# finegrain-ai/refiners

Hardware: NVIDIA B200
Metric: SDXL 1024^2 bf16 denoising steps/s (latent batch 8, CFG, Euler) (higher is better)
Workload: dtype bf16

## Files before the change

### refiners_b200/csrc/tc_attention2.cu

```cuda
#include <cuda.h>

#include <cstdlib>

#include "common.cuh"
#include "tc_ptx.cuh"

namespace rb200 {
namespace {

using namespace ptx;

constexpr int QT = 128;
constexpr int KT = 128;
constexpr int HD = 64;
constexpr int STAGES = 2;
constexpr int NUM_THREADS = 640;
constexpr int Q_TILE_BYTES = QT * HD * 2;
constexpr int Q_BYTES = 2 * Q_TILE_BYTES;
constexpr int K_BYTES = KT * HD * 2, V_BYTES = KT * HD * 2;
constexpr int P_SLAB = QT * 64 * 2;
constexpr int P_BYTES = 2 * P_SLAB;
constexpr int TMEM_COLS = 512;
constexpr int XCHG_BYTES = 2  * 2  * 2  * QT * 4;
constexpr size_t SMEM_BYTES = 2 * Q_BYTES + STAGES * (K_BYTES + V_BYTES) + 2 * P_BYTES + 1024  + 256  + XCHG_BYTES;
static_assert(SMEM_BYTES <= 227 * 1024, "exceeds the 227 KB of shared memory a CTA can opt in to");
constexpr float RESCALE_LOG2 = 8.0f;

struct Attn2Params {
  void* o;
  int64_t o_sb, o_ss;
  int H;
  int64_t Sq, Sk;
  int n_pairs;
  int64_t total_work;
  int ntiles;
  float scale_log2e;
  uint32_t idesc_qk, idesc_pv;
  int d_out;
  int stagger;
};

template <typename T> __device__ __forceinline__ uint32_t pack2(float a, float b);
template <> __device__ __forceinline__ uint32_t pack2<__nv_bfloat16>(float a, float b) {
  __nv_bfloat162 v = __floats2bfloat162_rn(a, b);
  return *reinterpret_cast<uint32_t*>(&v);
}
template <> __device__ __forceinline__ uint32_t pack2<__half>(float a, float b) {
  __half2 v = __floats2half2_rn(a, b);
  return *reinterpret_cast<uint32_t*>(&v);
}

template <typename T, int POLY>
__global__ void __launch_bounds__(NUM_THREADS, 1)
tc_sdpa2_kernel(const __grid_constant__ CUtensorMap map_q, const __grid_constant__ CUtensorMap map_k,
                const __grid_constant__ CUtensorMap map_v, const Attn2Params p) {
  extern __shared__ uint8_t smem_raw[];
  uint8_t* smem = reinterpret_cast<uint8_t*>((reinterpret_cast<uintptr_t>(smem_raw) + 1023) & ~uintptr_t(1023));
  uint8_t* sQ = smem;
  uint8_t* sK = sQ + 2 * Q_BYTES;
  uint8_t* sV = sK + STAGES * K_BYTES;
  uint8_t* sP = sV + STAGES * V_BYTES;
  uint64_t* bars = reinterpret_cast<uint64_t*>(sP + 2 * P_BYTES);
  uint64_t* kv_full = bars;
  uint64_t* kv_empty = bars + STAGES;
  uint64_t* q_full = bars + 2 * STAGES;
  uint64_t* q_empty = q_full + 2;
  uint64_t* bar_s = q_full + 4;
  uint64_t* bar_sfree = q_full + 6;
  uint64_t* bar_p = q_full + 8;
  uint64_t* bar_o = q_full + 10;
  uint64_t* bar_ofree = q_full + 12;
  uint32_t* tmem_slot = reinterpret_cast<uint32_t*>(q_full + 14);
  float* xchg = reinterpret_cast<float*>(reinterpret_cast<uint8_t*>(bars) + 256);

  const int warp = threadIdx.x >> 5, lane = threadIdx.x & 31;
  const int wg = warp >> 2;

  if (warp == 0 && lane == 0) {
    prefetch_tmap(&map_q);
    prefetch_tmap(&map_k);
    prefetch_tmap(&map_v);
    for (int s = 0; s < STAGES; ++s) {
      mbar_init(&kv_full[s], 1);
      mbar_init(&kv_empty[s], 2);
    }
    for (int b = 0; b < 2; ++b) {
      mbar_init(&q_full[b], 1);
      mbar_init(&q_empty[b], 2);
      mbar_init(&bar_s[b], 1);
      mbar_init(&bar_sfree[b], 8);
      mbar_init(&bar_p[b], 8);
      mbar_init(&bar_o[b], 1);
      mbar_init(&bar_ofree[b], 8);
    }
    fence_barrier_init();
  }
  if (warp == 1) tmem_alloc<TMEM_COLS>(tmem_slot);
  tcgen05_fence_before();
  __syncthreads();
  tcgen05_fence_after();
  const uint32_t tmem_base = *tmem_slot;

  if (wg == 0) {
    setmaxnreg_dec<56>();
    if (warp == 0) {
      if (lane == 0) {
        int stage = 0;
        uint32_t phase = 0;
        uint32_t n = 0;
        for (int64_t w = blockIdx.x; w < p.total_work; w += gridDim.x, ++n) {
          const int pair = int(w % p.n_pairs);
          const int h = int((w / p.n_pairs) % p.H);
          const int b = int(w / (int64_t(p.n_pairs) * p.H));
          const uint32_t qb = n & 1, qph = (n >> 1) & 1;
          mbar_wait(&q_empty[qb], qph ^ 1, 1);
          mbar_arrive_expect_tx(&q_full[qb], Q_BYTES);
          tma_load_4d(sQ + qb * Q_BYTES, &map_q, &q_full[qb], 0, h, pair * 2 * QT, b);
          tma_load_4d(sQ + qb * Q_BYTES + Q_TILE_BYTES, &map_q, &q_full[qb], 0, h, pair * 2 * QT + QT, b);
          for (int j = 0; j < p.ntiles; ++j) {
            mbar_wait(&kv_empty[stage], phase ^ 1, 2);
            mbar_arrive_expect_tx(&kv_full[stage], K_BYTES + V_BYTES);
            tma_load_4d(sK + stage * K_BYTES, &map_k, &kv_full[stage], 0, h, j * KT, b);
            tma_load_4d(sV + stage * V_BYTES, &map_v, &kv_full[stage], 0, h, j * KT, b);
            if (++stage == STAGES) {
              stage = 0;
              phase ^= 1;
            }
          }
        }
      }
    } else if (warp == 1 || warp == 2) {
      if (lane == 0) {
        const int g = warp - 1;
        int st_k = 0, st_v = 0;
        uint32_t ph_k = 0;
        uint32_t t = 0;
        uint32_t s_issued = 0;
        uint32_t n = 0;
        const uint32_t tmem_s = tmem_base + g * 128, tmem_o = tmem_base + 256 + g * 64;
        const uint32_t pbase = smem_u32(sP + g * P_BYTES);
        auto issue_s = [&](uint32_t qb, int stage_k) {
          if (s_issued > 0) mbar_wait(&bar_sfree[g], (s_issued - 1) & 1, 4);
          ++s_issued;
          tcgen05_fence_after();
          const uint64_t dq = desc_kmajor(smem_u32(sQ + qb * Q_BYTES + g * Q_TILE_BYTES));
          const uint64_t dk = desc_kmajor(smem_u32(sK + stage_k * K_BYTES));
#pragma unroll
          for (int k = 0; k < HD / 16; ++k) umma_f16(tmem_s, dq + uint64_t(k * 2), dk + uint64_t(k * 2), p.idesc_qk, k > 0);
          umma_commit(&bar_s[g]);
        };
        auto next_k = [&]() {
          if (++st_k == STAGES) {
            st_k = 0;
            ph_k ^= 1;
          }
        };
        for (int64_t w = blockIdx.x; w < p.total_work; w += gridDim.x, ++n) {
          const uint32_t qb = n & 1, qph = (n >> 1) & 1;
          mbar_wait(&q_full[qb], qph, 5);
          mbar_wait(&kv_full[st_k], ph_k, 3);
          issue_s(qb, st_k);
          next_k();
          for (int j = 0; j < p.ntiles; ++j) {
            if (j + 1 < p.ntiles) {
              mbar_wait(&kv_full[st_k], ph_k, 6);
              issue_s(qb, st_k);
              next_k();
            }
            mbar_wait(&bar_p[g], t & 1, 7);
            if (j == 0 && n > 0) mbar_wait(&bar_ofree[g], (n - 1) & 1, 8);
            tcgen05_fence_after();
            const uint32_t vbase = smem_u32(sV + st_v * V_BYTES);
#pragma unroll
            for (int k = 0; k < KT / 16; ++k) {
              const uint64_t dp = desc_kmajor(pbase + (k >> 2) * P_SLAB) + uint64_t((k & 3) * 2);
              const uint64_t dv = desc_mnmajor(vbase, V_BYTES) + uint64_t(k * 128);
              umma_f16(tmem_o, dp, dv, p.idesc_pv, (j > 0 || k > 0) ? 1u : 0u);
            }
            umma_commit(&kv_empty[st_v]);
            umma_commit(&bar_o[g]);
            ++t;
            if (++st_v == STAGES) st_v = 0;
          }
          umma_commit(&q_empty[qb]);
        }
      }
    }
  } else {
    setmaxnreg_inc<104>();
    const int g = (wg - 1) >> 1;
    const int hf = (wg - 1) & 1;
    const int lg = warp & 3;
    const int row = lg * 32 + lane;
    const uint32_t lane_off = uint32_t(lg * 32) << 16;
    const uint32_t tmem_s = tmem_base + g * 128 + hf * 64 + lane_off;
    const uint32_t tmem_o = tmem_base + 256 + g * 64 + hf * 32 + lane_off;
    const uint32_t prow = smem_u32(sP + g * P_BYTES + hf * P_SLAB + row * 128);
    const int sw = row & 7;
    const uint32_t xg = smem_u32(xchg + g * (2 * 2 * QT));
    const uint32_t x_mine = xg + uint32_t(hf * QT + row) * 4, x_other = xg + uint32_t((hf ^ 1) * QT + row) * 4;
    const uint32_t a_s = smem_u32(&bar_s[g]), a_sfree = smem_u32(&bar_sfree[g]), a_p = smem_u32(&bar_p[g]);
    const uint32_t a_o = smem_u32(&bar_o[g]), a_ofree = smem_u32(&bar_ofree[g]);
    const uint32_t swz = uint32_t(sw) << 4;
    const uint32_t xbar = 1 + g;
    T* obase = static_cast<T*>(p.o);
    uint32_t t = 0;
    uint32_t n = 0;
    for (int64_t w = blockIdx.x; w < p.total_work; w += gridDim.x, ++n) {
      const int pair = int(w % p.n_pairs);
      const int h = int((w / p.n_pairs) % p.H);
      const int64_t b = w / (int64_t(p.n_pairs) * p.H);
      float m_run = -INFINITY, l_run = 0.f;
      for (int j = 0; j < p.ntiles; ++j, ++t) {
        mbar_wait_a(a_s, t & 1);
        tcgen05_fence_after();
        float s[KT / 2];
        {
          uint32_t r0[32], r1[32];
          tmem_ld_32x32(tmem_s, r0);
          tmem_ld_32x32(tmem_s + 32, r1);
          tmem_ld_wait();
#pragma unroll
          for (int i = 0; i < 32; ++i) {
            s[i] = __uint_as_float(r0[i]);
            s[32 + i] = __uint_as_float(r1[i]);
          }
        }
        tcgen05_fence_before();
        __syncwarp();
        if (lane == 0) mbar_arrive_relaxed_a(a_sfree);
        const int64_t left = p.Sk - int64_t(j) * KT - hf * 64;
        if (left < 64) {
          const int valid = left > 0 ? int(left) : 0;
#pragma unroll
          for (int i = 0; i < 64; ++i)
            if (i >= valid) s[i] = -INFINITY;
        }
        float tm0 = fmaxf(s[0], s[1]), tm1 = fmaxf(s[2], s[3]), tm2 = fmaxf(s[4], s[5]), tm3 = fmaxf(s[6], s[7]);
#pragma unroll
        for (int i = 8; i < 64; i += 8) {
          tm0 = fmaxf(tm0, fmaxf(s[i], s[i + 1]));
          tm1 = fmaxf(tm1, fmaxf(s[i + 2], s[i + 3]));
          tm2 = fmaxf(tm2, fmaxf(s[i + 4], s[i + 5]));
          tm3 = fmaxf(tm3, fmaxf(s[i + 6], s[i + 7]));
        }
        const uint32_t slot = (t & 1) * (2 * QT * 4);
        const float mine = fmaxf(fmaxf(tm0, tm1), fmaxf(tm2, tm3));
        st_shared_f32(x_mine + slot, mine);
        named_bar_sync(xbar, 256);
        const float tmax = fmaxf(mine, ld_shared_f32(x_other + slot));
        bool waited_o = false;
        if (j == 0) {
          m_run = tmax;
        } else {
          const float m_new = fmaxf(m_run, tmax);
          const bool grew = (m_new - m_run) * p.scale_log2e > RESCALE_LOG2;
          if (__any_sync(0xffffffffu, grew)) {
            mbar_wait_a(a_o, (t - 1) & 1);
            waited_o = true;
            tcgen05_fence_after();
            const float alpha = ex2_approx((m_run - m_new) * p.scale_log2e);
            uint32_t raw[32];
            tmem_ld_32x32(tmem_o, raw);
            tmem_ld_wait();
#pragma unroll
            for (int i = 0; i < 32; ++i) raw[i] = __float_as_uint(__uint_as_float(raw[i]) * alpha);
            tmem_st_32x32(tmem_o, raw);
            tmem_st_wait();
            l_run *= alpha;
            m_run = m_new;
          }
        }
        const float mb = m_run * p.scale_log2e;
        if ((j > 0 && !waited_o) || (j == 0 && t > 0)) mbar_wait_a(a_o, (t - 1) & 1);
        if (p.stagger == 1) {
          if (g == 1 && j == 0) named_bar_sync(3, 512);
        } else if (p.stagger == 2) {
          if (g == 1) named_bar_sync(3, 512);
          else if (t > 0) named_bar_sync(4, 512);
        }
        const uint64_t sc2 = f32x2(p.scale_log2e, p.scale_log2e), nmb2 = f32x2(-mb, -mb);
        uint64_t sum_a = f32x2(0.f, 0.f), sum_b = sum_a;
#pragma unroll
        for (int c = 0; c < 8; ++c) {
          uint32_t pk[4];
#pragma unroll
          for (int q = 0; q < 2; ++q) {
            const int i = c * 8 + q * 4;
            float x0, x1, x2, x3;
            f32x2_split(fma_f32x2(f32x2(s[i], s[i + 1]), sc2, nmb2), x0, x1);
            f32x2_split(fma_f32x2(f32x2(s[i + 2], s[i + 3]), sc2, nmb2), x2, x3);
            const float p0 = ex2_approx(x0), p2 = ex2_approx(x2);
            const float p1 = POLY >= 2 ? ex2_poly(x1) : ex2_approx(x1);
            const float p3 = POLY >= 1 ? ex2_poly(x3) : ex2_approx(x3);
            sum_a = add_f32x2(sum_a, f32x2(p0, p1));
            sum_b = add_f32x2(sum_b, f32x2(p2, p3));
            pk[q * 2] = pack2<T>(p0, p1);
            pk[q * 2 + 1] = pack2<T>(p2, p3);
          }
          st_shared_v4(prow + ((uint32_t(c) << 4) ^ swz), pk[0], pk[1], pk[2], pk[3]);
        }
        {
          float a0, a1;
          f32x2_split(add_f32x2(sum_a, sum_b), a0, a1);
          l_run += a0 + a1;
        }
        if (p.stagger == 1) {
          if (g == 0 && j == 0) named_bar_arrive(3, 512);
        } else if (p.stagger == 2) {
          named_bar_arrive(g == 0 ? 3 : 4, 512);
        }
        fence_proxy_async();
        tcgen05_fence_before();
        __syncwarp();
        if (lane == 0) mbar_arrive_a(a_p);
      }
      const uint32_t slot = (t & 1) * (2 * QT * 4);
      st_shared_f32(x_mine + slot, l_run);
      named_bar_sync(xbar, 256);
      const float l_row = l_run + ld_shared_f32(x_other + slot);
      named_bar_sync(xbar, 256);
      mbar_wait_a(a_o, (t - 1) & 1);
      tcgen05_fence_after();
      const float inv = l_row > 0.f ? 1.f / l_row : 0.f;
      float acc[32];
      {
        uint32_t raw[32];
        tmem_ld_32x32(tmem_o, raw);
        tmem_ld_wait();
#pragma unroll
        for (int i = 0; i < 32; ++i) acc[i] = inv * __uint_as_float(raw[i]);
      }
      tcgen05_fence_before();
      __syncwarp();
      if (lane == 0) mbar_arrive_relaxed_a(a_ofree);
      const int64_t qi = (int64_t(pair) * 2 + g) * QT + row;
      if (qi < p.Sq) {
        T* dst = obase + b * p.o_sb + qi * p.o_ss + int64_t(h) * p.d_out + hf * 32;
        if ((reinterpret_cast<uintptr_t>(dst) & 15) == 0 && (p.d_out & 7) == 0) {
#pragma unroll
          for (int c = 0; c < 4; ++c) {
            if (hf * 32 + c * 8 >= p.d_out) break;
            uint4 v;
            v.x = pack2<T>(acc[c * 8], acc[c * 8 + 1]);
            v.y = pack2<T>(acc[c * 8 + 2], acc[c * 8 + 3]);
            v.z = pack2<T>(acc[c * 8 + 4], acc[c * 8 + 5]);
            v.w = pack2<T>(acc[c * 8 + 6], acc[c * 8 + 7]);
            reinterpret_cast<uint4*>(dst)[c] = v;
          }
        } else {
#pragma unroll
          for (int i = 0; i < 32; ++i)
            if (hf * 32 + i < p.d_out) dst[i] = from_f<T>(acc[i]);
        }
      }
    }
  }

  tcgen05_fence_before();
  __syncthreads();
  if (warp == 1) {
    tcgen05_fence_after();
    tmem_dealloc<TMEM_COLS>(tmem_base);
  }
}

typedef CUresult (*EncodeTiledFn)(CUtensorMap*, CUtensorMapDataType, cuuint32_t, void*, const cuuint64_t*, const cuuint64_t*,
                                  const cuuint32_t*, const cuuint32_t*, CUtensorMapInterleave, CUtensorMapSwizzle,
                                  CUtensorMapL2promotion, CUtensorMapFloatOOBfill);
EncodeTiledFn encode_fn() {
  static EncodeTiledFn fn = [] {
    void* sym = nullptr;
    cudaDriverEntryPointQueryResult q;
    if (cudaGetDriverEntryPoint("cuTensorMapEncodeTiled", &sym, cudaEnableDefault, &q) != cudaSuccess || q != cudaDriverEntryPointSuccess)
      return EncodeTiledFn(nullptr);
    return reinterpret_cast<EncodeTiledFn>(sym);
  }();
  return fn;
}

int make_map(CUtensorMap* map, int dtype, const void* base, int64_t B, int64_t S, int H, int64_t sb, int64_t ss, int D) {
  EncodeTiledFn fn = encode_fn();
  if (!fn) RB200_FAIL(-4, "cuTensorMapEncodeTiled unavailable");
  const cuuint64_t dims[4] = {cuuint64_t(D), cuuint64_t(H), cuuint64_t(S), cuuint64_t(B)};
  const cuuint64_t strides[3] = {cuuint64_t(D) * 2, cuuint64_t(ss) * 2, cuuint64_t(sb) * 2};
  const cuuint32_t box[4] = {64, 1, 128, 1};
  const cuuint32_t es[4] = {1, 1, 1, 1};
  const CUtensorMapDataType dt = dtype == RB200_BF16 ? CU_TENSOR_MAP_DATA_TYPE_BFLOAT16 : CU_TENSOR_MAP_DATA_TYPE_FLOAT16;
  CUresult rc = fn(map, dt, 4, const_cast<void*>(base), dims, strides, box, es, CU_TENSOR_MAP_INTERLEAVE_NONE,
                   CU_TENSOR_MAP_SWIZZLE_128B, CU_TENSOR_MAP_L2_PROMOTION_L2_256B, CU_TENSOR_MAP_FLOAT_OOB_FILL_NONE);
  if (rc != CUDA_SUCCESS) RB200_FAIL(-4, "sdpa2 tensor map encode failed (%d): S=%lld H=%d ss=%lld sb=%lld", int(rc), (long long)S, H, (long long)ss, (long long)sb);
  return 0;
}

bool ok_operand(const void* ptr, int64_t sb, int64_t ss) {
  return (reinterpret_cast<uintptr_t>(ptr) & 15) == 0 && ss % 8 == 0 && sb % 8 == 0;
}

template <typename T, int POLY>
int launch(cudaStream_t st, const CUtensorMap& mq, const CUtensorMap& mk, const CUtensorMap& mv, const Attn2Params& prm) {
  static PerDeviceOnce configured;
  if (configured.needed()) {
    if (cudaFuncSetAttribute(tc_sdpa2_kernel<T, POLY>, cudaFuncAttributeMaxDynamicSharedMemorySize, int(SMEM_BYTES)) != cudaSuccess)
      RB200_FAIL(-2, "tc_sdpa2: cannot reserve %zu bytes of shared memory", SMEM_BYTES);
    configured.done();
  }
  const int64_t cap = sm_count();
  const int grid = int(prm.total_work < cap ? prm.total_work : cap);
  tc_sdpa2_kernel<T, POLY><<<grid, NUM_THREADS, SMEM_BYTES, st>>>(mq, mk, mv, prm);
  RB200_CHECK_LAUNCH("tc_sdpa2");
  return 0;
}

int env_int(const char* name, int fallback) {
  const char* e = getenv(name);
  return e ? atoi(e) : fallback;
}

}

bool tc_sdpa2_supported(const SdpaProblem& p) {
  static const int enabled = env_int("RB200_ATTN_V2", 1);
  if (!enabled) return false;
  if (p.dtype != RB200_BF16 && p.dtype != RB200_FP16) return false;
  if (p.D < 8 || p.D > 64 || (p.D & 7) != 0 || p.causal) return false;
  if (p.bias_h != nullptr || (p.k2 != nullptr && p.Sk2 > 0)) return false;
  if (p.Sq <= QT || p.Sk <= KT || p.B < 1) return false;
  return ok_operand(p.q, p.q_sb, p.q_ss) && ok_operand(p.k, p.k_sb, p.k_ss) && ok_operand(p.v, p.v_sb, p.v_ss);
}

int tc_sdpa2(cudaStream_t st, const SdpaProblem& p) {
  CUtensorMap mq, mk, mv;
  if (int rc = make_map(&mq, p.dtype, p.q, p.B, p.Sq, p.H, p.q_sb, p.q_ss, p.D)) return rc;
  if (int rc = make_map(&mk, p.dtype, p.k, p.B, p.Sk, p.H, p.k_sb, p.k_ss, p.D)) return rc;
  if (int rc = make_map(&mv, p.dtype, p.v, p.B, p.Sk, p.H, p.v_sb, p.v_ss, p.D)) return rc;
  Attn2Params prm{};
  prm.o = p.o;
  prm.o_sb = p.o_sb;
  prm.o_ss = p.o_ss;
  prm.H = p.H;
  prm.Sq = p.Sq;
  prm.Sk = p.Sk;
  prm.n_pairs = int(ceil_div(p.Sq, 2 * QT));
  prm.total_work = int64_t(prm.n_pairs) * p.H * p.B;
  prm.ntiles = int(ceil_div(p.Sk, KT));
  prm.scale_log2e = p.scale * 1.4426950408889634f;
  const uint32_t fmt = p.dtype == RB200_BF16 ? 1u : 0u;
  const uint32_t common = (1u << 4) | (fmt << 7) | (fmt << 10) | (uint32_t(QT >> 4) << 24);
  prm.idesc_qk = common | (uint32_t(KT >> 3) << 17);
  prm.idesc_pv = common | (uint32_t(HD >> 3) << 17) | (1u << 16);
  prm.d_out = p.D;
  static const int stagger = env_int("RB200_ATTN_STAGGER", 2);
  prm.stagger = stagger;
  static const int poly = env_int("RB200_ATTN_POLY", 0);
  const bool bf = p.dtype == RB200_BF16;
  if (poly >= 2) return bf ? launch<__nv_bfloat16, 2>(st, mq, mk, mv, prm) : launch<__half, 2>(st, mq, mk, mv, prm);
  if (poly == 1) return bf ? launch<__nv_bfloat16, 1>(st, mq, mk, mv, prm) : launch<__half, 1>(st, mq, mk, mv, prm);
  return bf ? launch<__nv_bfloat16, 0>(st, mq, mk, mv, prm) : launch<__half, 0>(st, mq, mk, mv, prm);
}

}
```

### refiners_b200/csrc/tc_ptx.cuh

```cuda
#pragma once

#include <cuda.h>
#include <stdint.h>


namespace rb200 {
namespace ptx {

static __device__ __forceinline__ uint32_t smem_u32(const void* p) { return static_cast<uint32_t>(__cvta_generic_to_shared(p)); }

static __device__ __forceinline__ void mbar_init(uint64_t* bar, uint32_t count) {
  asm volatile("mbarrier.init.shared::cta.b64 [%0], %1;" ::"r"(smem_u32(bar)), "r"(count));
}
static __device__ __forceinline__ void fence_barrier_init() { asm volatile("fence.mbarrier_init.release.cluster;" ::: "memory"); }
static __device__ __forceinline__ void mbar_arrive_expect_tx(uint64_t* bar, uint32_t bytes) {
  asm volatile("mbarrier.arrive.expect_tx.shared::cta.b64 _, [%0], %1;" ::"r"(smem_u32(bar)), "r"(bytes) : "memory");
}
static __device__ __forceinline__ void mbar_arrive(uint64_t* bar) {
  asm volatile("mbarrier.arrive.shared::cta.b64 _, [%0];" ::"r"(smem_u32(bar)) : "memory");
}
static __device__ __forceinline__ void mbar_arrive_relaxed(uint64_t* bar) {
  asm volatile("mbarrier.arrive.relaxed.cta.shared::cta.b64 _, [%0];" ::"r"(smem_u32(bar)) : "memory");
}
static __device__ __forceinline__ bool mbar_try_wait(uint64_t* bar, uint32_t parity) {
  uint32_t ok;
  asm volatile(
      "{\n\t.reg .pred p;\n\t"
      "mbarrier.try_wait.parity.shared::cta.b64 p, [%1], %2;\n\t"
      "selp.u32 %0, 1, 0, p;\n\t}"
      : "=r"(ok)
      : "r"(smem_u32(bar)), "r"(parity)
      : "memory");
  return ok != 0;
}
static __device__ __forceinline__ void mbar_wait(uint64_t* bar, uint32_t parity, int tag = 0) {
  (void)tag;
  for (uint32_t spin = 0; !mbar_try_wait(bar, parity); ++spin) {
    if (spin > (1u << 26)) __trap();
  }
}

static __device__ __forceinline__ void mbar_arrive_a(uint32_t bar) {
  asm volatile("mbarrier.arrive.shared::cta.b64 _, [%0];" ::"r"(bar) : "memory");
}
static __device__ __forceinline__ void mbar_arrive_relaxed_a(uint32_t bar) {
  asm volatile("mbarrier.arrive.relaxed.cta.shared::cta.b64 _, [%0];" ::"r"(bar) : "memory");
}
static __device__ __forceinline__ bool mbar_try_wait_a(uint32_t bar, uint32_t parity) {
  uint32_t ok;
  asm volatile(
      "{\n\t.reg .pred p;\n\t"
      "mbarrier.try_wait.parity.shared::cta.b64 p, [%1], %2;\n\t"
      "selp.u32 %0, 1, 0, p;\n\t}"
      : "=r"(ok)
      : "r"(bar), "r"(parity)
      : "memory");
  return ok != 0;
}
static __device__ __forceinline__ void mbar_wait_a(uint32_t bar, uint32_t parity) {
  for (uint32_t spin = 0; !mbar_try_wait_a(bar, parity); ++spin) {
    if (spin > (1u << 26)) __trap();
  }
}
static __device__ __forceinline__ float ld_shared_f32(uint32_t addr) {
  float v;
  asm volatile("ld.shared.f32 %0, [%1];" : "=f"(v) : "r"(addr) : "memory");
  return v;
}
static __device__ __forceinline__ void st_shared_f32(uint32_t addr, float v) {
  asm volatile("st.shared.f32 [%0], %1;" ::"r"(addr), "f"(v) : "memory");
}

static __device__ __forceinline__ uint64_t f32x2(float lo, float hi) {
  uint64_t r;
  asm("mov.b64 %0, {%1, %2};" : "=l"(r) : "f"(lo), "f"(hi));
  return r;
}
static __device__ __forceinline__ void f32x2_split(uint64_t v, float& lo, float& hi) {
  asm("mov.b64 {%0, %1}, %2;" : "=f"(lo), "=f"(hi) : "l"(v));
}
static __device__ __forceinline__ uint64_t fma_f32x2(uint64_t a, uint64_t b, uint64_t c) {
  uint64_t d;
  asm("fma.rn.f32x2 %0, %1, %2, %3;" : "=l"(d) : "l"(a), "l"(b), "l"(c));
  return d;
}
static __device__ __forceinline__ uint64_t add_f32x2(uint64_t a, uint64_t b) {
  uint64_t d;
  asm("add.rn.f32x2 %0, %1, %2;" : "=l"(d) : "l"(a), "l"(b));
  return d;
}

static __device__ __forceinline__ void prefetch_tmap(const CUtensorMap* map) {
  asm volatile("prefetch.tensormap [%0];" ::"l"(reinterpret_cast<uint64_t>(map)) : "memory");
}
static __device__ __forceinline__ void tma_load_4d(void* dst, const CUtensorMap* map, uint64_t* bar, int c0, int c1, int c2, int c3) {
  asm volatile(
      "cp.async.bulk.tensor.4d.shared::cluster.global.mbarrier::complete_tx::bytes [%0], [%1, {%3, %4, %5, %6}], [%2];"
      ::"r"(smem_u32(dst)), "l"(reinterpret_cast<uint64_t>(map)), "r"(smem_u32(bar)), "r"(c0), "r"(c1), "r"(c2), "r"(c3)
      : "memory");
}
static __device__ __forceinline__ void fence_proxy_async() { asm volatile("fence.proxy.async.shared::cta;" ::: "memory"); }

static __device__ __forceinline__ void tcgen05_fence_before() { asm volatile("tcgen05.fence::before_thread_sync;" ::: "memory"); }
static __device__ __forceinline__ void tcgen05_fence_after() { asm volatile("tcgen05.fence::after_thread_sync;" ::: "memory"); }

template <int COLS>
static __device__ __forceinline__ void tmem_alloc(uint32_t* dst_smem) {
  asm volatile("tcgen05.alloc.cta_group::1.sync.aligned.shared::cta.b32 [%0], %1;" ::"r"(smem_u32(dst_smem)), "n"(COLS) : "memory");
  asm volatile("tcgen05.relinquish_alloc_permit.cta_group::1.sync.aligned;" ::: "memory");
}
template <int COLS>
static __device__ __forceinline__ void tmem_dealloc(uint32_t addr) {
  asm volatile("tcgen05.dealloc.cta_group::1.sync.aligned.b32 %0, %1;" ::"r"(addr), "n"(COLS) : "memory");
}

static __device__ __forceinline__ void umma_f16(uint32_t tmem_d, uint64_t desc_a, uint64_t desc_b, uint32_t idesc, uint32_t accumulate) {
  asm volatile(
      "{\n\t.reg .pred p;\n\t"
      "setp.ne.b32 p, %4, 0;\n\t"
      "tcgen05.mma.cta_group::1.kind::f16 [%0], %1, %2, %3, p;\n\t}"
      ::"r"(tmem_d), "l"(desc_a), "l"(desc_b), "r"(idesc), "r"(accumulate)
      : "memory");
}
static __device__ __forceinline__ void umma_commit(uint64_t* bar) {
  asm volatile("tcgen05.commit.cta_group::1.mbarrier::arrive::one.shared::cluster.b64 [%0];" ::"r"(smem_u32(bar)) : "memory");
}

static __device__ __forceinline__ void tmem_ld_32x32(uint32_t taddr, uint32_t (&r)[32]) {
  asm volatile(
      "tcgen05.ld.sync.aligned.32x32b.x32.b32 "
      "{%0, %1, %2, %3, %4, %5, %6, %7, %8, %9, %10, %11, %12, %13, %14, %15, "
      "%16, %17, %18, %19, %20, %21, %22, %23, %24, %25, %26, %27, %28, %29, %30, %31}, [%32];"
      : "=r"(r[0]), "=r"(r[1]), "=r"(r[2]), "=r"(r[3]), "=r"(r[4]), "=r"(r[5]), "=r"(r[6]), "=r"(r[7]), "=r"(r[8]),
        "=r"(r[9]), "=r"(r[10]), "=r"(r[11]), "=r"(r[12]), "=r"(r[13]), "=r"(r[14]), "=r"(r[15]), "=r"(r[16]),
        "=r"(r[17]), "=r"(r[18]), "=r"(r[19]), "=r"(r[20]), "=r"(r[21]), "=r"(r[22]), "=r"(r[23]), "=r"(r[24]),
        "=r"(r[25]), "=r"(r[26]), "=r"(r[27]), "=r"(r[28]), "=r"(r[29]), "=r"(r[30]), "=r"(r[31])
      : "r"(taddr)
      : "memory");
}
static __device__ __forceinline__ void tmem_ld_32x16(uint32_t taddr, uint32_t (&r)[16]) {
  asm volatile(
      "tcgen05.ld.sync.aligned.32x32b.x16.b32 "
      "{%0, %1, %2, %3, %4, %5, %6, %7, %8, %9, %10, %11, %12, %13, %14, %15}, [%16];"
      : "=r"(r[0]), "=r"(r[1]), "=r"(r[2]), "=r"(r[3]), "=r"(r[4]), "=r"(r[5]), "=r"(r[6]), "=r"(r[7]), "=r"(r[8]),
        "=r"(r[9]), "=r"(r[10]), "=r"(r[11]), "=r"(r[12]), "=r"(r[13]), "=r"(r[14]), "=r"(r[15])
      : "r"(taddr)
      : "memory");
}
static __device__ __forceinline__ void tmem_ld_wait() { asm volatile("tcgen05.wait::ld.sync.aligned;" ::: "memory"); }
static __device__ __forceinline__ void tmem_st_32x32(uint32_t taddr, const uint32_t (&r)[32]) {
  asm volatile(
      "tcgen05.st.sync.aligned.32x32b.x32.b32 [%0], "
      "{%1, %2, %3, %4, %5, %6, %7, %8, %9, %10, %11, %12, %13, %14, %15, %16, "
      "%17, %18, %19, %20, %21, %22, %23, %24, %25, %26, %27, %28, %29, %30, %31, %32};"
      ::"r"(taddr), "r"(r[0]), "r"(r[1]), "r"(r[2]), "r"(r[3]), "r"(r[4]), "r"(r[5]), "r"(r[6]), "r"(r[7]), "r"(r[8]), "r"(r[9]),
        "r"(r[10]), "r"(r[11]), "r"(r[12]), "r"(r[13]), "r"(r[14]), "r"(r[15]), "r"(r[16]), "r"(r[17]), "r"(r[18]), "r"(r[19]),
        "r"(r[20]), "r"(r[21]), "r"(r[22]), "r"(r[23]), "r"(r[24]), "r"(r[25]), "r"(r[26]), "r"(r[27]), "r"(r[28]), "r"(r[29]),
        "r"(r[30]), "r"(r[31])
      : "memory");
}
static __device__ __forceinline__ void tmem_st_wait() { asm volatile("tcgen05.wait::st.sync.aligned;" ::: "memory"); }

static __device__ __forceinline__ uint64_t desc_kmajor(uint32_t addr) {
  return uint64_t((addr >> 4) & 0x3FFF) | (uint64_t(1024 >> 4) << 32) | (uint64_t(1) << 46) | (uint64_t(2) << 61);
}
static __device__ __forceinline__ uint64_t desc_mnmajor(uint32_t addr, uint32_t tile_bytes) {
  return uint64_t((addr >> 4) & 0x3FFF) | (uint64_t((tile_bytes >> 4) & 0x3FFF) << 16) | (uint64_t(1024 >> 4) << 32) |
         (uint64_t(1) << 46) | (uint64_t(2) << 61);
}

static __device__ __forceinline__ float ex2_approx(float x) {
  float y;
  asm("ex2.approx.ftz.f32 %0, %1;" : "=f"(y) : "f"(x));
  return y;
}
static __device__ __forceinline__ float ex2_poly(float x) {
  x = fmaxf(x, -126.0f);
  const float t = x + 12582912.0f;
  const float f = x - (t - 12582912.0f);
  float p = fmaf(f, 0.0551716648f, 0.2426111251f);
  p = fmaf(p, f, 0.6932609677f);
  p = fmaf(p, f, 0.9999280572f);
  return __int_as_float(__float_as_int(p) + (__float_as_int(t) << 23));
}

static __device__ __forceinline__ void named_bar_sync(uint32_t id, uint32_t threads) {
  asm volatile("bar.sync %0, %1;" ::"r"(id), "r"(threads) : "memory");
}
static __device__ __forceinline__ void named_bar_arrive(uint32_t id, uint32_t threads) {
  asm volatile("bar.arrive %0, %1;" ::"r"(id), "r"(threads) : "memory");
}
static __device__ __forceinline__ void st_shared_v4(uint32_t addr, uint32_t a, uint32_t b, uint32_t c, uint32_t d) {
  asm volatile("st.shared.v4.b32 [%0], {%1, %2, %3, %4};" ::"r"(addr), "r"(a), "r"(b), "r"(c), "r"(d) : "memory");
}

template <int N>
static __device__ __forceinline__ void setmaxnreg_inc() { asm volatile("setmaxnreg.inc.sync.aligned.u32 %0;" ::"n"(N)); }
template <int N>
static __device__ __forceinline__ void setmaxnreg_dec() { asm volatile("setmaxnreg.dec.sync.aligned.u32 %0;" ::"n"(N)); }

}
}
```

Baseline: 7.659.

## Stage softmax P in tensor memory and use TMEM-operand MMA for PV

The softmax warps now write P into a dedicated tensor-memory region with tcgen05.st instead of swizzled stores to shared memory. The PV MMA takes its A operand straight from TMEM through a new TS-form umma wrapper. Freeing the shared-memory P buffers allows the K/V pipeline to grow from 2 to 4 stages, and the default stagger mode changes from 2 to 1. The wait for the previous PV now sits just before the TMEM store, which adds a synchronisation dependency on P reuse and relies on the TMEM A-operand layout being right.

```diff
diff --git a/refiners_b200/csrc/tc_attention2.cu b/refiners_b200/csrc/tc_attention2.cu
--- a/refiners_b200/csrc/tc_attention2.cu
+++ b/refiners_b200/csrc/tc_attention2.cu
@@ -13,16 +13,15 @@
 constexpr int QT = 128;
 constexpr int KT = 128;
 constexpr int HD = 64;
-constexpr int STAGES = 2;
+constexpr int STAGES = 4;
 constexpr int NUM_THREADS = 640;
 constexpr int Q_TILE_BYTES = QT * HD * 2;
 constexpr int Q_BYTES = 2 * Q_TILE_BYTES;
 constexpr int K_BYTES = KT * HD * 2, V_BYTES = KT * HD * 2;
-constexpr int P_SLAB = QT * 64 * 2;
-constexpr int P_BYTES = 2 * P_SLAB;
 constexpr int TMEM_COLS = 512;
+constexpr int TMEM_P = 384;
 constexpr int XCHG_BYTES = 2  * 2  * 2  * QT * 4;
-constexpr size_t SMEM_BYTES = 2 * Q_BYTES + STAGES * (K_BYTES + V_BYTES) + 2 * P_BYTES + 1024  + 256  + XCHG_BYTES;
+constexpr size_t SMEM_BYTES = 2 * Q_BYTES + STAGES * (K_BYTES + V_BYTES) + 1024  + 256  + XCHG_BYTES;
 static_assert(SMEM_BYTES <= 227 * 1024, "exceeds the 227 KB of shared memory a CTA can opt in to");
 constexpr float RESCALE_LOG2 = 8.0f;
 
@@ -59,8 +58,7 @@
   uint8_t* sQ = smem;
   uint8_t* sK = sQ + 2 * Q_BYTES;
   uint8_t* sV = sK + STAGES * K_BYTES;
-  uint8_t* sP = sV + STAGES * V_BYTES;
-  uint64_t* bars = reinterpret_cast<uint64_t*>(sP + 2 * P_BYTES);
+  uint64_t* bars = reinterpret_cast<uint64_t*>(sV + STAGES * V_BYTES);
   uint64_t* kv_full = bars;
   uint64_t* kv_empty = bars + STAGES;
   uint64_t* q_full = bars + 2 * STAGES;
@@ -137,8 +135,7 @@
         uint32_t t = 0;
         uint32_t s_issued = 0;
         uint32_t n = 0;
-        const uint32_t tmem_s = tmem_base + g * 128, tmem_o = tmem_base + 256 + g * 64;
-        const uint32_t pbase = smem_u32(sP + g * P_BYTES);
+        const uint32_t tmem_s = tmem_base + g * 128, tmem_o = tmem_base + 256 + g * 64, tmem_p = tmem_base + TMEM_P + g * 64;
         auto issue_s = [&](uint32_t qb, int stage_k) {
           if (s_issued > 0) mbar_wait(&bar_sfree[g], (s_issued - 1) & 1, 4);
           ++s_issued;
@@ -173,9 +170,8 @@
             const uint32_t vbase = smem_u32(sV + st_v * V_BYTES);
 #pragma unroll
             for (int k = 0; k < KT / 16; ++k) {
-              const uint64_t dp = desc_kmajor(pbase + (k >> 2) * P_SLAB) + uint64_t((k & 3) * 2);
               const uint64_t dv = desc_mnmajor(vbase, V_BYTES) + uint64_t(k * 128);
-              umma_f16(tmem_o, dp, dv, p.idesc_pv, (j > 0 || k > 0) ? 1u : 0u);
+              umma_f16_ts(tmem_o, tmem_p + k * 8, dv, p.idesc_pv, (j > 0 || k > 0) ? 1u : 0u);
             }
             umma_commit(&kv_empty[st_v]);
             umma_commit(&bar_o[g]);
@@ -195,13 +191,11 @@
     const uint32_t lane_off = uint32_t(lg * 32) << 16;
     const uint32_t tmem_s = tmem_base + g * 128 + hf * 64 + lane_off;
     const uint32_t tmem_o = tmem_base + 256 + g * 64 + hf * 32 + lane_off;
-    const uint32_t prow = smem_u32(sP + g * P_BYTES + hf * P_SLAB + row * 128);
-    const int sw = row & 7;
+    const uint32_t tmem_p = tmem_base + TMEM_P + g * 64 + hf * 32 + lane_off;
     const uint32_t xg = smem_u32(xchg + g * (2 * 2 * QT));
     const uint32_t x_mine = xg + uint32_t(hf * QT + row) * 4, x_other = xg + uint32_t((hf ^ 1) * QT + row) * 4;
     const uint32_t a_s = smem_u32(&bar_s[g]), a_sfree = smem_u32(&bar_sfree[g]), a_p = smem_u32(&bar_p[g]);
     const uint32_t a_o = smem_u32(&bar_o[g]), a_ofree = smem_u32(&bar_ofree[g]);
-    const uint32_t swz = uint32_t(sw) << 4;
     const uint32_t xbar = 1 + g;
     T* obase = static_cast<T*>(p.o);
     uint32_t t = 0;
@@ -272,7 +266,6 @@
           }
         }
         const float mb = m_run * p.scale_log2e;
-        if ((j > 0 && !waited_o) || (j == 0 && t > 0)) mbar_wait_a(a_o, (t - 1) & 1);
         if (p.stagger == 1) {
           if (g == 1 && j == 0) named_bar_sync(3, 512);
         } else if (p.stagger == 2) {
@@ -281,24 +274,20 @@
         }
         const uint64_t sc2 = f32x2(p.scale_log2e, p.scale_log2e), nmb2 = f32x2(-mb, -mb);
         uint64_t sum_a = f32x2(0.f, 0.f), sum_b = sum_a;
-#pragma unroll
-        for (int c = 0; c < 8; ++c) {
-          uint32_t pk[4];
-#pragma unroll
-          for (int q = 0; q < 2; ++q) {
-            const int i = c * 8 + q * 4;
-            float x0, x1, x2, x3;
-            f32x2_split(fma_f32x2(f32x2(s[i], s[i + 1]), sc2, nmb2), x0, x1);
-            f32x2_split(fma_f32x2(f32x2(s[i + 2], s[i + 3]), sc2, nmb2), x2, x3);
-            const float p0 = ex2_approx(x0), p2 = ex2_approx(x2);
-            const float p1 = POLY >= 2 ? ex2_poly(x1) : ex2_approx(x1);
-            const float p3 = POLY >= 1 ? ex2_poly(x3) : ex2_approx(x3);
-            sum_a = add_f32x2(sum_a, f32x2(p0, p1));
-            sum_b = add_f32x2(sum_b, f32x2(p2, p3));
-            pk[q * 2] = pack2<T>(p0, p1);
-            pk[q * 2 + 1] = pack2<T>(p2, p3);
-          }
-          st_shared_v4(prow + ((uint32_t(c) << 4) ^ swz), pk[0], pk[1], pk[2], pk[3]);
+        uint32_t pk[KT / 4];
+#pragma unroll
+        for (int q = 0; q < KT / 8; ++q) {
+          const int i = q * 4;
+          float x0, x1, x2, x3;
+          f32x2_split(fma_f32x2(f32x2(s[i], s[i + 1]), sc2, nmb2), x0, x1);
+          f32x2_split(fma_f32x2(f32x2(s[i + 2], s[i + 3]), sc2, nmb2), x2, x3);
+          const float p0 = ex2_approx(x0), p2 = ex2_approx(x2);
+          const float p1 = POLY >= 2 ? ex2_poly(x1) : ex2_approx(x1);
+          const float p3 = POLY >= 1 ? ex2_poly(x3) : ex2_approx(x3);
+          sum_a = add_f32x2(sum_a, f32x2(p0, p1));
+          sum_b = add_f32x2(sum_b, f32x2(p2, p3));
+          pk[q * 2] = pack2<T>(p0, p1);
+          pk[q * 2 + 1] = pack2<T>(p2, p3);
         }
         {
           float a0, a1;
@@ -310,7 +299,10 @@
         } else if (p.stagger == 2) {
           named_bar_arrive(g == 0 ? 3 : 4, 512);
         }
-        fence_proxy_async();
+        if (j > 0 && !waited_o) mbar_wait_a(a_o, (t - 1) & 1);
+        tcgen05_fence_after();
+        tmem_st_32x32(tmem_p, pk);
+        tmem_st_wait();
         tcgen05_fence_before();
         __syncwarp();
         if (lane == 0) mbar_arrive_a(a_p);
@@ -450,7 +442,7 @@
   prm.idesc_qk = common | (uint32_t(KT >> 3) << 17);
   prm.idesc_pv = common | (uint32_t(HD >> 3) << 17) | (1u << 16);
   prm.d_out = p.D;
-  static const int stagger = env_int("RB200_ATTN_STAGGER", 2);
+  static const int stagger = env_int("RB200_ATTN_STAGGER", 1);
   prm.stagger = stagger;
   static const int poly = env_int("RB200_ATTN_POLY", 0);
   const bool bf = p.dtype == RB200_BF16;
diff --git a/refiners_b200/csrc/tc_ptx.cuh b/refiners_b200/csrc/tc_ptx.cuh
--- a/refiners_b200/csrc/tc_ptx.cuh
+++ b/refiners_b200/csrc/tc_ptx.cuh
@@ -120,6 +120,14 @@
       "setp.ne.b32 p, %4, 0;\n\t"
       "tcgen05.mma.cta_group::1.kind::f16 [%0], %1, %2, %3, p;\n\t}"
       ::"r"(tmem_d), "l"(desc_a), "l"(desc_b), "r"(idesc), "r"(accumulate)
+      : "memory");
+}
+static __device__ __forceinline__ void umma_f16_ts(uint32_t tmem_d, uint32_t tmem_a, uint64_t desc_b, uint32_t idesc, uint32_t accumulate) {
+  asm volatile(
+      "{\n\t.reg .pred p;\n\t"
+      "setp.ne.b32 p, %4, 0;\n\t"
+      "tcgen05.mma.cta_group::1.kind::f16 [%0], [%1], %2, %3, p;\n\t}"
+      ::"r"(tmem_d), "r"(tmem_a), "l"(desc_b), "r"(idesc), "r"(accumulate)
       : "memory");
 }
 static __device__ __forceinline__ void umma_commit(uint64_t* bar) {
```

Result: faster. 7.863 (median of 6 runs) (+2.7%).
